# STLABTW/ST-DADK

Hardware: NVIDIA B200
Metric: train_samples_per_s (higher is better)
Workload: dtype tf32

## Files before the change

st_dadk_b200/csrc/api.cu:

```cuda
#include <cstdarg>
#include <cstdio>
#include <cstring>

#include "layer.cuh"
#include "misc.cuh"
#include "sparse.cuh"
#include "predict.cuh"
#include "field.cuh"

using namespace stdadk;

static thread_local char g_err[512] = "";

static int fail(int code, const char* fmt, ...) {
    va_list ap;
    va_start(ap, fmt);
    vsnprintf(g_err, sizeof(g_err), fmt, ap);
    va_end(ap);
    return code;
}
static int check_launch(const char* what) {
    cudaError_t e = cudaGetLastError();
    if (e != cudaSuccess) return fail((int)e, "%s: %s", what, cudaGetErrorString(e));
    return 0;
// ... 715 lines not shown
    K->p_cov = a->p_cov;
    K->fn = a->basis_fn;
    return 0;
}

static int make_groups(int n_groups, const int64_t* group_end, int64_t n, GroupsP* G) {
    REQUIRE(n_groups >= 1 && n_groups <= 8 && group_end, "optimizer: 1..8 parameter groups supported, got %d", n_groups);
    int64_t prev = 0;
    for (int i = 0; i < n_groups; ++i) {
        REQUIRE(group_end[i] >= prev, "optimizer: group_end must be non-decreasing");
        G->end[i] = prev = group_end[i];
    }
    REQUIRE(prev == n, "optimizer: last group_end (%lld) != n (%lld)", (long long)prev, (long long)n);
    G->n = n_groups;
    return 0;
}

size_t stdadk_celllist_ws_bytes(int32_t k_s, int32_t n_levels) {
    if (k_s < 0 || n_levels < 1 || n_levels > SP_MAX_LEVELS) return 0;
    return celllist_bytes(k_s, n_levels);
}

int stdadk_celllist_build(const float* knots4, int32_t k_s, const int32_t* level_begin, int32_t n_levels, void* ws,
                          size_t ws_bytes, void* stream) {
    if (int r = check_device()) return r;
    REQUIRE(knots4 && level_begin && ws && k_s >= 1, "celllist_build: NULL argument / no knots");
    REQUIRE(n_levels >= 1 && n_levels <= SP_MAX_LEVELS, "celllist_build: 1..%d levels, got %d", SP_MAX_LEVELS, n_levels);
    REQUIRE(((reinterpret_cast<uintptr_t>(ws) | reinterpret_cast<uintptr_t>(knots4)) & 15) == 0,
            "celllist_build: knots4 / workspace must be 16-byte aligned");
    REQUIRE(ws_bytes >= celllist_bytes(k_s, n_levels), "celllist_build: workspace of %zu B, need %zu B", ws_bytes,
            celllist_bytes(k_s, n_levels));
    CellBuildK K{};
    K.knots = reinterpret_cast<const float4*>(knots4);
    K.k_s = k_s;
    K.n_levels = n_levels;
    for (int l = 0; l <= n_levels; ++l) {
        REQUIRE(level_begin[l] >= (l ? level_begin[l - 1] : 0) && level_begin[l] <= k_s, "celllist_build: level_begin not monotone");
        K.level_begin[l] = level_begin[l];
    }
    REQUIRE(level_begin[0] == 0 && level_begin[n_levels] == k_s, "celllist_build: levels must cover [0, k_s)");
    K.ws = static_cast<int*>(ws);
    size_t ib = (celllist_ints(k_s, n_levels) * 4 + 15) & ~(size_t)15;
    K.sorted = reinterpret_cast<float4*>(static_cast<uint8_t*>(ws) + ib);
    celllist_build_kernel<<<1, CL_THREADS, 0, (cudaStream_t)stream>>>(K);
    return check_launch("celllist_build");
}

size_t stdadk_sqnorm_ws_floats(void) { return (size_t)SQNORM_BLOCKS * 8 + 8; }

int stdadk_grad_sqnorm(const float* g, int64_t n, int n_groups, const int64_t* group_end, float* sqnorms,
                       float* workspace, void* stream) {
    if (int r = check_device()) return r;
    REQUIRE(g && sqnorms && workspace && n > 0, "grad_sqnorm: bad arguments (workspace of stdadk_sqnorm_ws_floats() "
            "zero-initialised floats is required)");
    REQUIRE((reinterpret_cast<uintptr_t>(g) & 15) == 0, "grad_sqnorm: g must be 16-byte aligned");
    GroupsP G{};
    if (int r = make_groups(n_groups, group_end, n, &G)) return r;
    long long blocks = ((n >> 2) + SQNORM_THREADS * 4 - 1) / (SQNORM_THREADS * 4);
    if (blocks < 1) blocks = 1;
    if (blocks > SQNORM_BLOCKS) blocks = SQNORM_BLOCKS;
    sqnorm_kernel<<<(int)blocks, SQNORM_THREADS, 0, (cudaStream_t)stream>>>(g, n, G, sqnorms, workspace);
    return check_launch("grad_sqnorm");
}

int stdadk_sparse_l1_fwd(const stdadk_sparse_args* a, void* stream) {
    if (int r = check_device()) return r;
    SparseK K{};
    if (int r = sparse_fill(a, &K, false)) return r;
    if (a->pts.n_rows <= 0) return 0;
    int blocks = grid_for(a->pts.n_rows, SP_WARPS, 8);
    sparse_spatial_fwd_kernel<<<blocks, SP_WARPS * 32, 0, (cudaStream_t)stream>>>(K);
    return check_launch("sparse_l1_fwd");
}

int stdadk_sparse_l1_wgrad(const stdadk_sparse_args* a, void* stream) {
    if (int r = check_device()) return r;
    SparseK K{};
    if (int r = sparse_fill(a, &K, true)) return r;
    if (a->pts.n_rows <= 0) return 0;
    int blocks = grid_for(a->pts.n_rows, SP_WARPS, 8);
    sparse_spatial_wgrad_kernel<<<blocks, SP_WARPS * 32, 0, (cudaStream_t)stream>>>(K);
    return check_launch("sparse_l1_wgrad");
}

__global__ void step_inc_kernel(int* c) { *c += 1; }

int stdadk_peer_allreduce(const stdadk_peer_allreduce_args* a, void* stream) {
    if (int r = check_device()) return r;
    REQUIRE(a && a->g && a->step_count, "peer_allreduce: NULL argument");
    REQUIRE(a->world >= 2 && a->world <= PEER_MAX && a->rank >= 0 && a->rank < a->world,
            "peer_allreduce: world=%d rank=%d outside [2,%d]", a->world, a->rank, PEER_MAX);
    REQUIRE(a->n > 0 && a->n % 4 == 0, "peer_allreduce: n=%lld must be a positive multiple of 4", (long long)a->n);
    static_assert(PEER_MAX == STDADK_MAX_PEERS, "peer limits differ");
    REQUIRE((reinterpret_cast<uintptr_t>(a->g) & 15) == 0, "peer_allreduce: g must be 16-byte aligned");
    PeerK K{};
    for (int r = 0; r < a->world; ++r) {
        REQUIRE(a->recv[r] && (reinterpret_cast<uintptr_t>(a->recv[r]) & 15) == 0,
                "peer_allreduce: rank %d receive area not mapped / not 16-byte aligned", r);
        K.recv[r] = static_cast<uint4*>(a->recv[r]);
    }
    K.g = a->g;
    K.n2 = a->n / 2;
    K.step_count = a->step_count;
    K.rank = a->rank;
    K.world = a->world;
    REQUIRE(a->mode >= 0 && a->mode <= 2, "peer_allreduce: mode=%d (0 automatic, 1 one-shot, 2 two-phase)", a->mode);
    K.two_phase = a->mode == 2 || (a->mode == 0 && a->world >= 4);
    if (a->n_groups > 0) {
        REQUIRE(a->group_end && a->sqnorms && a->workspace, "peer_allreduce: fused norm needs group_end / sqnorms / workspace");
        K.n_norm = a->group_end[a->n_groups - 1];
        REQUIRE(K.n_norm <= a->n, "peer_allreduce: norm range exceeds n");
        if (int r = make_groups(a->n_groups, a->group_end, K.n_norm, &K.G)) return r;
        K.sq_out = a->sqnorms;
        K.ws = a->workspace;
    }
    long long blocks = (K.n2 + PEER_THREADS * 2 - 1) / (PEER_THREADS * 2);
    if (blocks > 148) blocks = 148;
    if (blocks < 1) blocks = 1;
    peer_allreduce_kernel<<<(int)blocks, PEER_THREADS, 0, (cudaStream_t)stream>>>(K);
    return check_launch("peer_allreduce");
}

int stdadk_adamw_ema_step(const stdadk_adamw_args* a, void* stream) {
    if (int r = check_device()) return r;
    REQUIRE(a && a->p && a->g && a->m && a->v && a->hyper && a->step_count && a->n > 0, "adamw: bad arguments");
    AdamK K{};
    if (int r = make_groups(a->n_groups, a->group_end, a->n, &K.G)) return r;
    K.p = a->p;
    K.g = a->g;
    K.m = a->m;
    K.v = a->v;
    K.shadow = a->shadow;
    K.n = a->n;
    K.hyper = a->hyper;
    K.sqnorms = a->sqnorms;
    K.step_count = a->step_count;
    K.beta1 = a->beta1;
    K.beta2 = a->beta2;
    K.eps = a->eps;
    K.ema_decay = a->ema_decay;
    K.g_zero = a->zero_grad ? const_cast<float*>(a->g) : nullptr;
    K.loss_acc = a->loss_acc;
    K.loss_sum = a->loss_sum;
    K.loss_last = a->loss_last;
    REQUIRE(((reinterpret_cast<uintptr_t>(a->p) | reinterpret_cast<uintptr_t>(a->g) | reinterpret_cast<uintptr_t>(a->m) |
              reinterpret_cast<uintptr_t>(a->v) | reinterpret_cast<uintptr_t>(a->shadow)) & 15) == 0,
            "adamw: buffers must be 16-byte aligned");
    if (a->fuse_norm) {
        REQUIRE(a->norm_ws, "adamw: fuse_norm needs norm_ws");
        K.sq_out = const_cast<float*>(a->sqnorms);
        K.norm_ws = a->norm_ws;
        K.step_rw = a->step_count;
        long long blocks = ((a->n + 3) / 4 + 255) / 256;
        if (blocks > 148) blocks = 148;
        const int sms = g_sm_count > 0 ? g_sm_count : 148;
        if (blocks > sms) blocks = sms;
        if (blocks < 1) blocks = 1;
        adamw_ema_kernel<true><<<(int)blocks, 256, 0, (cudaStream_t)stream>>>(K);
        return check_launch("adamw_ema_step (fused tail)");
    }
    step_inc_kernel<<<1, 1, 0, (cudaStream_t)stream>>>(a->step_count);
    adamw_ema_kernel<false><<<grid_for((a->n + 3) / 4, 256, 8), 256, 0, (cudaStream_t)stream>>>(K);
    return check_launch("adamw_ema_step");
}

}
```

st_dadk_b200/csrc/misc.cuh:

```cuda
#pragma once
#include "common.cuh"

namespace stdadk {

__global__ void pack_image_kernel(const float* __restrict__ src, long long row_stride, long long col_stride,
                                  long long rows, long long cols, float* __restrict__ img, long long n_chunks,
                                  int slabs) {
    for (long long idx = blockIdx.x * (long long)blockDim.x + threadIdx.x; idx < n_chunks;
         idx += (long long)gridDim.x * blockDim.x) {
        int chunk = (int)(idx & 7);
        int row = (int)((idx >> 3) & 127);
        long long ts = idx >> 10;
        int slab = (int)(ts % slabs);
        long long tile = ts / slabs;
        long long r = tile * TILE_M + row;
        float v[4];
#pragma unroll
        for (int e = 0; e < 4; ++e) {
            long long c = (long long)slab * SLAB_K + chunk * 4 + e;
            v[e] = (r < rows && c < cols) ? to_tf32(src[r * row_stride + c * col_stride]) : 0.0f;
        }
        float* dst = img + ts * SLAB_FLOATS;
        *reinterpret_cast<float4*>(reinterpret_cast<uint8_t*>(dst) + swz_off((uint32_t)row, (uint32_t)chunk)) =
            make_float4(v[0], v[1], v[2], v[3]);
// ... 197 lines not shown
}
constexpr int PEER_THREADS = 256;
__device__ __forceinline__ void peer_two_phase(const PeerK& P, unsigned int epoch, long long par_off, long long i0,
                                               long long stride) {
    float2* g2 = reinterpret_cast<float2*>(P.g);
    const long long m = (P.n2 + P.world - 1) / P.world;
    const long long own_lo = (long long)P.rank * m, own_hi = min(P.n2, own_lo + m);
    const uint4* mine = P.recv[P.rank];
    for (long long i = i0; i < P.n2; i += stride) {
        if (i >= own_lo && i < own_hi) continue;
        const int owner = (int)(i / m);
        const float2 v = g2[i];
        uint4* dst = nullptr;
#pragma unroll
        for (int p = 0; p < PEER_MAX; ++p)
            if (p == owner) dst = P.recv[p];
        st_sys_v4(dst + (par_off + P.rank) * P.n2 + i, make_uint4(__float_as_uint(v.x), epoch, __float_as_uint(v.y), epoch));
    }
    for (long long i = i0; i < P.n2; i += stride) {
        if (i < own_lo || i >= own_hi) continue;
        const float2 own = g2[i];
        float2 sum = make_float2(0.0f, 0.0f);
#pragma unroll
        for (int s = 0; s < PEER_MAX; ++s)
            if (s < P.world) {
                const float2 v = s == P.rank ? own : peer_wait_packet(mine + (par_off + s) * P.n2 + i, epoch);
                sum.x += v.x;
                sum.y += v.y;
            }
        g2[i] = sum;
        const uint4 pkt = make_uint4(__float_as_uint(sum.x), epoch, __float_as_uint(sum.y), epoch);
#pragma unroll
        for (int p = 0; p < PEER_MAX; ++p)
            if (p < P.world && p != P.rank) st_sys_v4(P.recv[p] + (par_off + P.rank) * P.n2 + i, pkt);
    }
    for (long long i = i0; i < P.n2; i += stride) {
        if (i >= own_lo && i < own_hi) continue;
        const int owner = (int)(i / m);
        g2[i] = peer_wait_packet(mine + (par_off + owner) * P.n2 + i, epoch);
    }
}
__global__ void __launch_bounds__(PEER_THREADS) peer_allreduce_kernel(const __grid_constant__ PeerK P) {
    const unsigned int epoch = (unsigned int)(*P.step_count) + 1u;
    const long long par_off = (long long)(epoch & 1u) * P.world;
    const long long stride = (long long)gridDim.x * blockDim.x;
    const long long i0 = blockIdx.x * (long long)blockDim.x + threadIdx.x;
    float2* g2 = reinterpret_cast<float2*>(P.g);
    float acc[8];
#pragma unroll
    for (int k = 0; k < 8; ++k) acc[k] = 0.0f;
    if (P.two_phase) {
        peer_two_phase(P, epoch, par_off, i0, stride);
        if (P.G.n == 0) return;
        for (long long i = i0; i < P.n2; i += stride) {
            const float2 sum = g2[i];
            const long long e = i << 1;
            const float vv[2] = {sum.x, sum.y};
#pragma unroll
            for (int j = 0; j < 2; ++j)
                if (e + j < P.n_norm) {
                    const int gi = group_of(P.G, e + j);
#pragma unroll
                    for (int k = 0; k < 8; ++k)
                        if (k == gi) acc[k] = fmaf(vv[j], vv[j], acc[k]);
                }
        }
    } else {
    for (long long i = i0; i < P.n2; i += stride) {
        const float2 v = g2[i];
        const uint4 pkt = make_uint4(__float_as_uint(v.x), epoch, __float_as_uint(v.y), epoch);
#pragma unroll
        for (int p = 0; p < PEER_MAX; ++p)
            if (p < P.world && p != P.rank) st_sys_v4(P.recv[p] + (par_off + P.rank) * P.n2 + i, pkt);
    }
    const uint4* mine = P.recv[P.rank];
    for (long long i = i0; i < P.n2; i += stride) {
        const float2 own = g2[i];
        float2 sum = make_float2(0.0f, 0.0f);
#pragma unroll
        for (int s = 0; s < PEER_MAX; ++s)
            if (s < P.world) {
                float2 v = own;
                if (s != P.rank) v = peer_wait_packet(mine + (par_off + s) * P.n2 + i, epoch);
                sum.x += v.x;
                sum.y += v.y;
            }
        g2[i] = sum;
        if (P.G.n > 0) {
            const long long e = i << 1;
            const float vv[2] = {sum.x, sum.y};
#pragma unroll
            for (int j = 0; j < 2; ++j)
                if (e + j < P.n_norm) {
                    const int gi = group_of(P.G, e + j);
#pragma unroll
                    for (int k = 0; k < 8; ++k)
                        if (k == gi) acc[k] = fmaf(vv[j], vv[j], acc[k]);
                }
        }
    }
    }
    if (P.G.n == 0) return;
    __shared__ float wsum[PEER_THREADS / 32][8];
    __shared__ bool last;
    const int warp = threadIdx.x >> 5, lane = threadIdx.x & 31;
#pragma unroll
    for (int k = 0; k < 8; ++k) {
        float s = warp_sum(acc[k]);
        if (lane == 0) wsum[warp][k] = s;
    }
    __syncthreads();
    if (threadIdx.x < 8) {
        float s = 0.0f;
        for (int w = 0; w < PEER_THREADS / 32; ++w) s += wsum[w][threadIdx.x];
        P.ws[blockIdx.x * 8 + threadIdx.x] = s;
    }
    __threadfence();
    __syncthreads();
    if (threadIdx.x == 0) {
        unsigned int* ticket = reinterpret_cast<unsigned int*>(P.ws + gridDim.x * 8);
        unsigned int t = atomicAdd(ticket, 1u);
        last = (t == gridDim.x - 1);
        if (last) *ticket = 0u;
    }
    __syncthreads();
    if (last && threadIdx.x < P.G.n) {
        __threadfence();
        float s = 0.0f;
        for (unsigned int b = 0; b < gridDim.x; ++b) s += P.ws[b * 8 + threadIdx.x];
        P.sq_out[threadIdx.x] = s;
    }
}

struct AdamK {
    float* p;
    const float* g;
    float* m;
    float* v;
    float* shadow;
    long long n;
    GroupsP G;
    const float* hyper;
    const float* sqnorms;
    const int* step_count;
    float beta1, beta2, eps, ema_decay;
    float* g_zero;
    float* loss_acc;
    float* loss_sum;
    float* loss_last;
    float* sq_out;
    float* norm_ws;
    int* step_rw;
};
template <bool FUSED>
__global__ void __launch_bounds__(256) adamw_ema_kernel(AdamK A) {
    __shared__ float s_sq[8];
    int step;
    if (FUSED) {
        step = *A.step_count + 1;
        float acc[8];
#pragma unroll
        for (int k = 0; k < 8; ++k) acc[k] = 0.0f;
        if (A.sqnorms) {
            const long long n4q = A.n >> 2;
            const float4* gq = reinterpret_cast<const float4*>(A.g);
            for (long long i = blockIdx.x * (long long)blockDim.x + threadIdx.x; i < n4q; i += (long long)gridDim.x * blockDim.x) {
                const float4 v = __ldg(gq + i);
                const long long e = i << 2;
                const float vv[4] = {v.x, v.y, v.z, v.w};
#pragma unroll
                for (int j = 0; j < 4; ++j) {
                    const int gi = group_of(A.G, e + j);
#pragma unroll
                    for (int k = 0; k < 8; ++k)
                        if (k == gi) acc[k] = fmaf(vv[j], vv[j], acc[k]);
                }
            }
            if (blockIdx.x == 0 && threadIdx.x < (A.n & 3)) {
                const long long i = (n4q << 2) + threadIdx.x;
                const float v = A.g[i];
                const int gi = group_of(A.G, i);
#pragma unroll
                for (int k = 0; k < 8; ++k)
                    if (k == gi) acc[k] = fmaf(v, v, acc[k]);
            }
        }
        __shared__ float wsum[8][8];
        const int warp = threadIdx.x >> 5, lane = threadIdx.x & 31;
#pragma unroll
        for (int k = 0; k < 8; ++k) {
            const float sk = warp_sum(acc[k]);
            if (lane == 0) wsum[warp][k] = sk;
        }
        __syncthreads();
        if (threadIdx.x < 8) {
            float sk = 0.0f;
            for (int w = 0; w < 8; ++w) sk += wsum[w][threadIdx.x];
            A.norm_ws[blockIdx.x * 8 + threadIdx.x] = sk;
        }
        __threadfence();
        __syncthreads();
        if (threadIdx.x == 0) {
            unsigned int* cnt = reinterpret_cast<unsigned int*>(A.norm_ws + gridDim.x * 8);
            volatile unsigned int* gen = cnt + 1;
            const unsigned int my_gen = *gen;
            if (atomicAdd(cnt, 1u) == gridDim.x - 1) {
                *cnt = 0u;
                __threadfence();
                atomicAdd(const_cast<unsigned int*>(gen), 1u);
            } else {
                long long t0 = clock64();
                while (*gen == my_gen) {
                    if (clock64() - t0 > 4000000000LL) __trap();
                }
            }
            __threadfence();
        }
        __syncthreads();
        if (threadIdx.x < 8) {
            float sk = 0.0f;
            for (unsigned int b = 0; b < gridDim.x; ++b) sk += __ldcg(&A.norm_ws[b * 8 + threadIdx.x]);
            s_sq[threadIdx.x] = sk;
            if (blockIdx.x == 0 && A.sq_out && threadIdx.x < A.G.n) A.sq_out[threadIdx.x] = sk;
        }
        if (blockIdx.x == 0 && threadIdx.x == 0) *A.step_rw = step;
        __syncthreads();
    } else {
        step = *A.step_count;
    }
    const float bc1 = 1.0f - powf(A.beta1, (float)step);
    const float bc2 = 1.0f - powf(A.beta2, (float)step);
    const float inv_sqrt_bc2 = 1.0f / sqrtf(bc2);
    float lr[8], wd[8], clip[8];
#pragma unroll
    for (int k = 0; k < 8; ++k) {
        lr[k] = wd[k] = 0.0f;
        clip[k] = 1.0f;
        if (k < A.G.n) {
            lr[k] = A.hyper[4 * k];
            wd[k] = A.hyper[4 * k + 1];
            float mx = A.hyper[4 * k + 2];
            if (A.sqnorms && mx > 0.0f) clip[k] = fminf(1.0f, mx / (sqrtf(FUSED ? s_sq[k] : A.sqnorms[k]) + 1e-6f));
        }
    }
    auto update = [&](long long i, float g, float& p, float& m, float& v, float& sh) {
        int gi = group_of(A.G, i);
        float l = lr[0], w = wd[0], c = clip[0];
#pragma unroll
        for (int k = 1; k < 8; ++k)
            if (k == gi) { l = lr[k]; w = wd[k]; c = clip[k]; }
        g *= c;
        p *= (1.0f - l * w);
        m = A.beta1 * m + (1.0f - A.beta1) * g;
        v = A.beta2 * v + (1.0f - A.beta2) * g * g;
        float denom = sqrtf(v) * inv_sqrt_bc2 + A.eps;
        p -= (l / bc1) * (m / denom);
        sh = A.ema_decay * sh + (1.0f - A.ema_decay) * p;
    };
    const long long n4 = A.n >> 2;
    const float4* g4 = reinterpret_cast<const float4*>(A.g);
    float4* p4 = reinterpret_cast<float4*>(A.p);
    float4* m4 = reinterpret_cast<float4*>(A.m);
    float4* v4 = reinterpret_cast<float4*>(A.v);
    float4* s4 = reinterpret_cast<float4*>(A.shadow);
    for (long long i = blockIdx.x * (long long)blockDim.x + threadIdx.x; i < n4;
         i += (long long)gridDim.x * blockDim.x) {
        float4 g = __ldg(g4 + i), p = p4[i], m = m4[i], v = v4[i];
        float4 sh = s4 ? s4[i] : make_float4(0.f, 0.f, 0.f, 0.f);
        const long long e = i << 2;
        update(e, g.x, p.x, m.x, v.x, sh.x);
        update(e + 1, g.y, p.y, m.y, v.y, sh.y);
        update(e + 2, g.z, p.z, m.z, v.z, sh.z);
        update(e + 3, g.w, p.w, m.w, v.w, sh.w);
        p4[i] = p;
        m4[i] = m;
        v4[i] = v;
        if (s4) s4[i] = sh;
        if (A.g_zero) reinterpret_cast<float4*>(A.g_zero)[i] = make_float4(0.f, 0.f, 0.f, 0.f);
    }
    if (blockIdx.x == 0 && threadIdx.x == 0 && A.loss_acc && A.loss_sum) {
        const float step_loss = *A.loss_acc;
        *A.loss_sum += step_loss;
        if (A.loss_last) *A.loss_last = step_loss;
        *A.loss_acc = 0.0f;
    }
    if (blockIdx.x == 0 && threadIdx.x < (A.n & 3)) {
        long long i = (n4 << 2) + threadIdx.x;
        float p = A.p[i], m = A.m[i], v = A.v[i], sh = A.shadow ? A.shadow[i] : 0.0f;
        update(i, A.g[i], p, m, v, sh);
        A.p[i] = p;
        A.m[i] = m;
        A.v[i] = v;
        if (A.shadow) A.shadow[i] = sh;
        if (A.g_zero) A.g_zero[i] = 0.0f;
    }
}

}
```

st_dadk_b200/trainer.py:

```python
from __future__ import annotations

import math
import os
import warnings
from dataclasses import dataclass
from typing import Dict, List, Optional

import numpy as np
import torch
import torch.distributed as dist

import threading

from . import _lib as L
from . import ops
from .executor import Executor, LossSpec, NetSpec


def _dist_on() -> bool:
    return dist.is_available() and dist.is_initialized() and dist.get_world_size() > 1


_CAPTURE_LOCK = threading.Lock()


class FlatState:

    def __init__(self, model, device):
        self.model = model
        blocks = model.hidden_blocks()
        entries = []
        for lin, ln in blocks:
            entries.append((lin.weight, (lin.in_features, lin.out_features), True))
            entries.append((lin.bias, tuple(lin.bias.shape), False))
            if ln is not None:
                entries.append((ln.weight, tuple(ln.weight.shape), False))
                entries.append((ln.bias, tuple(ln.bias.shape), False))
        if model.delta_params is not None:
            for d in model.delta_params:
                entries.append((d, tuple(d.shape), False))
        else:
            head = model.mlp[-1]
            entries.append((head.weight, tuple(head.weight.shape), False))
            entries.append((head.bias, tuple(head.bias.shape), False))
        n_mlp = sum(int(np.prod(s)) for _, s, _ in entries)
        sb = model.spatial_basis
        if sb.learnable:
            entries.append((sb.centers, tuple(sb.centers.shape), False))
            entries.append((sb.log_bandwidths, tuple(sb.log_bandwidths.shape), False))
        n = sum(int(np.prod(s)) for _, s, _ in entries)
        self.n = n
        self.group_end = [n_mlp, n] if sb.learnable else [n]
        q, d = model.output_dim, model.last_hidden_dim
        self.n_scratch = q * d + q if model.delta_params is not None else 0
        mk = lambda extra=0: torch.zeros(n + extra, dtype=torch.float32, device=device)
        self.p, self.m, self.v, self.shadow = mk(), mk(), mk(), mk()
        self.n_exchange = n + self.n_scratch + 1
        self.g = mk(self.n_scratch + 1 + (-self.n_exchange) % 4)
        self.loss_slot = self.g[n + self.n_scratch:n + self.n_scratch + 1]
        self.views: Dict[int, torch.Tensor] = {}
        self.gviews: Dict[int, torch.Tensor] = {}
        o = 0
        with torch.no_grad():
            for prm, shape, tr in entries:
                k = int(np.prod(shape))
                pv, gv = self.p[o:o + k].view(*shape), self.g[o:o + k].view(*shape)
                if tr:
                    pv, gv = pv.t(), gv.t()
                pv.copy_(prm.detach().to(device))
                prm.data = pv
                prm.grad = None
                self.views[id(prm)] = pv
                self.gviews[id(prm)] = gv
                o += k
        self.shadow.copy_(self.p)
        self._backup = None
        if self.n_scratch:
            self.g_head_w = self.g[n:n + q * d].view(q, d)
            self.g_head_b = self.g[n + q * d:n + q * d + q]

    def grad_views_for(self, model) -> dict:
        blocks = model.hidden_blocks()
        gv = self.gviews
        out = {"weights": [gv[id(l.weight)] for l, _ in blocks], "biases": [gv[id(l.bias)] for l, _ in blocks],
               "gammas": [gv[id(n.weight)] if n is not None else None for _, n in blocks],
               "betas": [gv[id(n.bias)] if n is not None else None for _, n in blocks]}
        if model.delta_params is not None:
            out["head_w"], out["head_b"] = self.g_head_w, self.g_head_b
        else:
            out["head_w"], out["head_b"] = gv[id(model.mlp[-1].weight)], gv[id(model.mlp[-1].bias)]
        sb = model.spatial_basis
        if sb.learnable:
            out["centers"], out["log_bandwidths"] = gv[id(sb.centers)], gv[id(sb.log_bandwidths)]
        else:
            out["centers"] = out["log_bandwidths"] = None
        return out

    def apply_shadow(self):
        self._backup = self.p.clone()
        self.p.copy_(self.shadow)

    def restore(self):
        self.p.copy_(self._backup)
        self._backup = None


@dataclass
class StepStats:
    loss: float
    n_rows: int


class Trainer:

    def __init__(self, model, config: dict, device, batches_per_epoch: int = 1, use_cuda_graph: bool = False):
        self.model = model.to(device)
        self.cfg = config
        if config.get("precision") is not None:
            self.model.precision = config["precision"]
        self.device = torch.device(device)
        if self.device.type != "cuda":
            raise RuntimeError("st_dadk_b200.Trainer runs on CUDA (sm_100) only; there is no CPU training path")
        self.flat = FlatState(self.model, self.device)
        self._peer = None
        if _dist_on() and dist.get_backend() == "nccl" and os.environ.get("STDADK_PEER_ALLREDUCE", "1") != "0":
            ok = torch.ones(1, device=self.device)
            try:
                from .peer import PeerExchange
                self._peer = PeerExchange(self.device, self.flat.n_exchange)
            except Exception as e:
                if "exceeds the peer-exchange limit" not in str(e):
                    warnings.warn(f"peer-memory gradient exchange unavailable ({e!r}); using the NCCL all-reduce")
                ok.zero_()
            dist.all_reduce(ok, op=dist.ReduceOp.MIN)
            if float(ok.item()) == 0.0:
                self._peer = None
        m = self.model
        self.learnable = bool(m.spatial_basis.learnable)
        self.q = m.output_dim
        self.head_w = torch.empty(self.q, m.last_hidden_dim, device=self.device)
        self.head_b = torch.empty(self.q, device=self.device)
        self.ex = Executor(self._spec())
        self.ex.loss_acc = self.flat.loss_slot
        self.ex.on_evict = lambda: self._graphs.clear()
        self.ex.alloc_grads(self.flat.g, self.flat.grad_views_for(m))
        self._init_loss()
        self._init_optimizer(batches_per_epoch)
        self.step_count = torch.zeros(1, dtype=torch.int32, device=self.device)
        self.sqnorms = torch.zeros(len(self.flat.group_end), device=self.device)
        self._sqnorm_ws = torch.zeros(L.lib().stdadk_sqnorm_ws_floats(), device=self.device)
        self._tail_ws = torch.zeros(148 * 8 + 8, device=self.device)
        self.seed = int(torch.initial_seed() & (2 ** 63 - 1))
        self.loss_sum = torch.zeros(1, device=self.device)
        self.loss_last = torch.zeros(1, device=self.device)
        self._g_clean = False
        self.use_cuda_graph = use_cuda_graph
        self._graphs: Dict[tuple, torch.cuda.CUDAGraph] = {}
        self._stage_idx = None
        self._host_stage = None
        self._host_perm = None
        self.world = dist.get_world_size() if _dist_on() else 1
        self.rank = dist.get_rank() if _dist_on() else 0
        c = self.cfg
        self._param_terms_possible = bool(
            self.learnable
            or (c.get("sparsity_penalty_type", "none") != "none"
                and (float(c.get("sparsity_lambda_l1", 0.001)) != 0.0 or float(c.get("sparsity_lambda_group", 0.01)) != 0.0))
            or (c.get("use_delta_reparameterization", False) and float(c.get("non_crossing_lambda", 0.0)) > 0))
        self.kernel_launches = 0

    def _spec(self) -> NetSpec:
        m = self.model
        self._refresh_head()
        return m.net_spec(self.head_w, self.head_b)

    def _refresh_head(self):
        m = self.model
        with torch.no_grad():
            if m.delta_params is not None:
                beta = torch.cumsum(torch.stack([d.detach() for d in m.delta_params]), dim=0)
                self.head_w.copy_(beta[:, 1:])
                self.head_b.copy_(beta[:, 0])
            else:
                self.head_w.copy_(m.mlp[-1].weight.detach())
                self.head_b.copy_(m.mlp[-1].bias.detach())

    def _init_loss(self):
        c = self.cfg
        rt = c.get("regression_type", "mean")
        if rt == "mean":
            self.loss = LossSpec("mse")
        elif rt == "quantile":
            if c.get("current_quantile") is None:
                raise ValueError("current_quantile must be specified for quantile regression")
            self.loss = LossSpec("pinball", [float(c["current_quantile"])])
        elif rt == "multi-quantile":
            taus = [float(x) for x in c.get("quantile_levels", [0.1, 0.5, 0.9])]
            ncw = 0.0 if c.get("use_delta_reparameterization", False) else float(c.get("non_crossing_weight", 0.0))
            self.loss = LossSpec("pinball", taus, ncw, int(c.get("non_crossing_power", 1)))
        else:
            raise ValueError(f"Unknown regression_type: {rt}")

    def _init_optimizer(self, batches_per_epoch: int):
        c = self.cfg
        self.lr = float(c.get("lr", 1e-3))
        self.wd = float(c.get("weight_decay", 1e-5))
        self.clip = float(c.get("grad_clip", 0) or 0)
        self.unfreeze_epoch = int(c.get("basis_unfreeze_epoch", 0))
        self.rampup_epochs = int(c.get("basis_lr_rampup_epochs", 0))
        dummy = lambda: [torch.nn.Parameter(torch.zeros(1))]
        if self.learnable:
            ratio = c.get("basis_lr_ratio", 0.05)
            init_basis = 0.0 if self.unfreeze_epoch > 0 else self.lr * ratio
            self.opt = torch.optim.AdamW([{"params": dummy(), "lr": self.lr, "name": "mlp"},
                                          {"params": dummy(), "lr": init_basis, "name": "basis"}], weight_decay=self.wd)
            for gq in self.opt.param_groups:
                gq["initial_lr"] = gq["lr"]
                if gq.get("name") == "basis":
                    gq["target_lr"] = self.lr * ratio
        else:
            self.opt = torch.optim.AdamW(dummy(), lr=self.lr, weight_decay=self.wd)
            for gq in self.opt.param_groups:
                gq["initial_lr"] = gq["lr"]
        self.batches_per_epoch = max(1, batches_per_epoch)
        self.warmup_epochs = int(c.get("warmup_epochs", 0))
        self.warmup_steps = self.warmup_epochs * self.batches_per_epoch if self.warmup_epochs > 0 else 0
        self.scheduler = None
        if c.get("scheduler") == "cosine":
            self.scheduler = torch.optim.lr_scheduler.CosineAnnealingLR(self.opt, T_max=c.get("epochs", 100),
                                                                        eta_min=self.lr * 0.5)
        self.ema_decay = 1.0 - 1.0 / (10.0 * self.batches_per_epoch)
        self.global_step = 0
        ng = len(self.opt.param_groups)
        self._hyper_ring = [torch.zeros(ng, 4, dtype=torch.float32).pin_memory() for _ in range(self.HYPER_SLOTS)]
        self._hyper_ev = [None] * self.HYPER_SLOTS
        self._hyper_k = 0
        self._hyper_last = None
        self.hyper = torch.zeros(ng, 4, dtype=torch.float32, device=self.device)

    HYPER_SLOTS = 16

    def _hyper_values(self):
        rows = []
        for gq in self.opt.param_groups:
            clip = self.clip * (0.1 if (self.learnable and gq.get("name") == "basis") else 1.0)
            rows.append((float(gq["lr"]), float(self.wd), float(clip)))
        return tuple(rows)

    def _push_hyper(self):
        vals = self._hyper_values()
        if vals == self._hyper_last:
            return
        k = self._hyper_k
        self._hyper_k = (k + 1) % self.HYPER_SLOTS
        if self._hyper_ev[k] is not None:
            self._hyper_ev[k].synchronize()
        slot = self._hyper_ring[k]
        for i, (lr, wd, clip) in enumerate(vals):
            slot[i, 0], slot[i, 1], slot[i, 2] = lr, wd, clip
        self.hyper.copy_(slot, non_blocking=True)
        ev = torch.cuda.Event()
        ev.record(torch.cuda.current_stream())
        self._hyper_ev[k] = ev
        self._hyper_last = vals

    def begin_epoch(self, epoch: int):
        if not (self.learnable and self.unfreeze_epoch > 0):
            return
        for gq in self.opt.param_groups:
            if gq.get("name") != "basis":
                continue
            if epoch == self.unfreeze_epoch:
                gq["lr"] = gq["target_lr"] * (0.1 if self.rampup_epochs > 0 else 1.0)
            elif self.unfreeze_epoch < epoch < self.unfreeze_epoch + self.rampup_epochs:
                gq["lr"] = gq["target_lr"] * (0.1 + 0.9 * (epoch - self.unfreeze_epoch) / self.rampup_epochs)

    def end_epoch(self, epoch: int):
        if self.scheduler is not None and epoch >= self.warmup_epochs:
            with warnings.catch_warnings():
                warnings.simplefilter("ignore")
                self.scheduler.step()

    def _penalty_terms(self):
        c, m = self.cfg, self.model
        terms = []
        if self.learnable:
            w = float(c.get("domain_penalty_weight", 0.0))
            if w > 0:
                terms.append(w * m.compute_domain_penalty())
            w = float(c.get("movement_penalty_weight", 0.0))
            if w > 0:
                terms.append(w * m.compute_movement_penalty())
        stype = c.get("sparsity_penalty_type", "none")
        l1, lg = float(c.get("sparsity_lambda_l1", 0.001)), float(c.get("sparsity_lambda_group", 0.01))
        if stype != "none" and (l1 != 0.0 or lg != 0.0):
            pen = m.compute_sparsity_penalty(penalty_type=stype, lambda_l1=l1, lambda_group=lg)
            if c.get("sparsity_apply_to_spatial", True):
                terms.append(pen["spatial_penalty"])
            if c.get("sparsity_apply_to_temporal", True):
                terms.append(pen["temporal_penalty"])
        if c.get("regression_type") == "multi-quantile" and c.get("use_delta_reparameterization", False):
            lam = float(c.get("non_crossing_lambda", 0.0))
            if lam > 0 and m.delta_params is not None and len(m.delta_params) > 1:
                pnc = 0.0
                for d in list(m.delta_params)[1:]:
                    pnc = pnc + d[0] - torch.max(d[0], torch.clamp(-d[1:], min=0.0).sum())
                terms.append(lam * pnc)
        return terms

    def _add_penalty_grads(self):
        terms = self._penalty_terms()
        if not terms:
            return None
        total = sum(terms)
        params = [p for p in self.model.parameters() if p.requires_grad]
        sb = self.model.spatial_basis
        sb._hook_enabled = False
        try:
            grads = torch.autograd.grad(total, params, allow_unused=True)
        finally:
            sb._hook_enabled = True
        for p, gr in zip(params, grads):
            if gr is not None:
                self.flat.gviews[id(p)].add_(gr)
        return total.detach()

    def _finish_special_grads(self):
        m = self.model
        if m.delta_params is not None:
            dbeta = torch.cat([self.flat.g_head_b[:, None], self.flat.g_head_w], dim=1)
            ddelta = torch.flip(torch.cumsum(torch.flip(dbeta, [0]), dim=0), [0])
            for k, d in enumerate(m.delta_params):
                self.flat.gviews[id(d)].copy_(ddelta[k])

    def _damp_center_grads(self):
        sb = self.model.spatial_basis
        if self.learnable and sb.gradient_damping:
            gv = self.flat.gviews[id(sb.centers)]
            gv.copy_(sb._damping_factor() * gv)

    def _step_compute(self, table, perm, row_begin: int, n_rows: int, global_rows: int, key_offset: int = 0):
        ex, fl = self.ex, self.flat
        if not self._g_clean:
            fl.g.zero_()
            ex.loss_acc.zero_()
        self._g_clean = False
        self._refresh_head()
        ex.prepare(force=True, for_backward=True)
        pts = ops.make_points(table.coords, table.t, table.X, index=perm, row_begin=row_begin, n_rows=n_rows)
        ex.forward(pts, train=True, seed=self.seed, y=table.y, loss=self.loss, inv_count=1.0 / (global_rows * self.q),
                   save=True, prepared=True, step_ptr=self.step_count, key_offset=key_offset)
        ex.backward(zero=False)
        self._finish_special_grads()

    def _step_exchange(self):
        if self.world > 1:
            if self._peer is not None:
                fuse = self._norm_fused()
                self._peer.allreduce(self.flat.g, self.step_count, self.flat.group_end if fuse else None, self.sqnorms)
            else:
                dist.all_reduce(self.flat.g[:self.flat.n_exchange])

    def _norm_fused(self) -> bool:
        return self._peer is not None and self.world > 1 and self.clip > 0 and not self._param_terms_possible

    def _step_update(self):
        ex, fl = self.ex, self.flat
        pen = self._add_penalty_grads()
        self._damp_center_grads()
        fused_tail = not self._norm_fused()
        scratch_tail = fl.n_scratch > 0
        ops.adamw_ema_step(fl.p, fl.g[:fl.n], fl.m, fl.v, fl.shadow, fl.group_end, self.hyper,
                           self.sqnorms if self.clip > 0 else None, self.step_count, ema_decay=self.ema_decay,
                           zero_grad=True, loss_acc=ex.loss_acc, loss_sum=self.loss_sum, loss_last=self.loss_last,
                           norm_ws=self._tail_ws if fused_tail else None)
        if scratch_tail:
            fl.g[fl.n:fl.n + fl.n_scratch].zero_()
        self._g_clean = True
        if pen is not None:
            self.loss_sum += pen

    def _step_body(self, table, perm, row_begin: int, n_rows: int, global_rows: int, key_offset: int = 0):
        self._step_compute(table, perm, row_begin, n_rows, global_rows, key_offset)
        self._step_exchange()
        self._step_update()

    def train_step(self, table, perm: torch.Tensor, row_begin: int, n_rows: int, global_rows: Optional[int] = None,
                   key_offset: Optional[int] = None):
        if global_rows is None:
            global_rows = n_rows
        if key_offset is None:
            key_offset = shard_rows(global_rows, self.rank, self.world)[0] if self.world > 1 else 0
        self._push_hyper()
        if self.use_cuda_graph:
            if self._stage_idx is None or self._stage_idx.shape[0] < n_rows:
                self._stage_idx = torch.zeros(max(n_rows, 1), dtype=torch.int64, device=self.device)
                self._graphs.clear()
            self._stage_idx[:n_rows].copy_(perm[row_begin:row_begin + n_rows])
            gkey = (n_rows, global_rows, table.coords.data_ptr(), table.t.data_ptr(), table.y.data_ptr(),
                    table.X.data_ptr() if table.X is not None else 0, key_offset)
            g = self._graphs.get(gkey)
            if g is None:
                with _CAPTURE_LOCK:
                    self._step_body(table, self._stage_idx, 0, n_rows, global_rows, key_offset)
                    torch.cuda.current_stream().synchronize()
                    mode = dict(capture_error_mode="thread_local")
                    one_graph = self.world == 1 or self._peer is not None
                    if one_graph:
                        g1 = torch.cuda.CUDAGraph()
                        with torch.cuda.graph(g1, **mode):
                            self._step_body(table, self._stage_idx, 0, n_rows, global_rows, key_offset)
                        g = (g1, None)
                    else:
                        g1, g2 = torch.cuda.CUDAGraph(), torch.cuda.CUDAGraph()
                        with torch.cuda.graph(g1, **mode):
                            self._step_compute(table, self._stage_idx, 0, n_rows, global_rows, key_offset)
                        with torch.cuda.graph(g2, **mode):
                            self._step_update()
                        g = (g1, g2)
                self._graphs[gkey] = g
            else:
                g[0].replay()
                if g[1] is not None:
                    self._step_exchange()
                    g[1].replay()
        else:
            self._step_body(table, perm, row_begin, n_rows, global_rows, key_offset)
        if self.global_step < self.warmup_steps:
            f = (self.global_step + 1) / self.warmup_steps
            for gq in self.opt.param_groups:
                gq["lr"] = gq["initial_lr"] * f
        self.global_step += 1

    def train_step_host(self, host_table, row_begin: int, n_rows: int, global_rows: Optional[int] = None,
                        lagged: bool = False) -> float:
        if self._host_stage is None or len(self._host_stage[0]) < n_rows:
            from stnf.dataio import ObservationTable
            z = lambda *sh: torch.zeros(*sh, dtype=torch.float32, device=self.device)
            mk = lambda: ObservationTable(z(n_rows, 2), z(n_rows), z(n_rows),
                                          z(n_rows, self.model.p) if self.model.p > 0 else None)
            self._host_stage = [mk(), mk()]
            self._graphs.clear()
            self._host_perm = torch.arange(n_rows, dtype=torch.int64, device=self.device)
            self._host_copy_stream = torch.cuda.Stream(device=self.device)
            self._host_ready = [torch.cuda.Event(), torch.cuda.Event()]
            self._host_done = [torch.cuda.Event(), torch.cuda.Event()]
            self._host_loss = [torch.full((1,), float("nan")).pin_memory(), torch.full((1,), float("nan")).pin_memory()]
            self._host_k = 0
            self._host_pending = None
            main = torch.cuda.current_stream()
            for e in self._host_done:
                e.record(main)
        k = self._host_k
        self._host_k ^= 1
        st = self._host_stage[k]
        sl = slice(row_begin, row_begin + n_rows)
        main = torch.cuda.current_stream()

        def copy_batch():
            st.coords[:n_rows].copy_(host_table.coords[sl], non_blocking=True)
            st.t[:n_rows].copy_(host_table.t[sl], non_blocking=True)
            st.y[:n_rows].copy_(host_table.y[sl], non_blocking=True)
            if st.X is not None:
                st.X[:n_rows].copy_(host_table.X[sl], non_blocking=True)

        if lagged or self._host_pending is not None:
            with torch.cuda.stream(self._host_copy_stream):
                self._host_copy_stream.wait_event(self._host_done[k])
                copy_batch()
                self._host_ready[k].record(self._host_copy_stream)
            main.wait_event(self._host_ready[k])
        else:
            copy_batch()
        self.train_step(st, self._host_perm, 0, n_rows, global_rows)
        self._host_loss[k].copy_(self.loss_last, non_blocking=True)
        self._host_done[k].record(main)
        prev, self._host_pending = self._host_pending, k
        if not lagged:
            self._host_done[k].synchronize()
            self._host_pending = None
            return float(self._host_loss[k].item())
        if prev is None:
            return float("nan")
        self._host_done[prev].synchronize()
        return float(self._host_loss[prev].item())

    def flush_host_loss(self) -> float:
        if self._host_pending is None:
            return float("nan")
        k, self._host_pending = self._host_pending, None
        self._host_done[k].synchronize()
        return float(self._host_loss[k].item())

    @property
    def launches_per_step(self) -> int:
        nh = self.ex.spec.n_hidden
        n = 1
        n += nh + nh + nh
        if self.learnable:
            n += 3
        n += 1 if not self._norm_fused() else 2
        if self._peer is not None and self.world > 1:
            n += 1
        return n

    def profile_step(self, table, perm, n_rows: int, global_rows: int, repeats: int = 10) -> dict:
        rec: List[tuple] = []
        saved = {}

        def wrap(name, fn, flops_of):
            def inner(*a, **k):
                e0, e1 = torch.cuda.Event(enable_timing=True), torch.cuda.Event(enable_timing=True)
                e0.record()
                r = fn(*a, **k)
                e1.record()
                rec.append((name(*a, **k) if callable(name) else name, e0, e1, flops_of(*a, **k)))
                return r
            return inner

        rows = float(n_rows)
        f_fwd = lambda a: 2.0 * rows * a.layer.n_in * a.layer.n_out
        f_bwd = lambda a: 2.0 * rows * a.layer.n_out * (a.layer.n_in + (a.n_next if not a.head else 0))
        f_wg = lambda a: 2.0 * rows * a.n_in * a.n_out
        patches = {
            "layer_fwd": (lambda a: f"layer_fwd[{a.layer.layer_id}]", f_fwd),
            "layer_bwd": (lambda a: f"layer_bwd[{a.layer.layer_id}]", f_bwd),
            "wgrad": (lambda a: f"wgrad[{a.n_in}x{a.n_out}]", f_wg),
            "knot_grad": ("knot_grad", lambda a: 2.0 * rows * a.n_out * self.model.k_spatial),
            "pack_image": ("pack_image", lambda *a, **k: 0.0),
            "pack_images": ("pack_images", lambda *a, **k: 0.0),
            "knots_prepare": ("knots_prepare", lambda *a, **k: 0.0),
            "tknots_prepare": ("knots_prepare", lambda *a, **k: 0.0),
            "grad_sqnorm": ("grad_sqnorm", lambda *a, **k: 0.0),
            "adamw_ema_step": ("adamw_ema_step", lambda *a, **k: 0.0),
        }
        use_graph, self.use_cuda_graph = self.use_cuda_graph, False
        try:
            for fname, (nm, fl) in patches.items():
                saved[fname] = getattr(ops, fname)
                setattr(ops, fname, wrap(nm, saved[fname], fl))
            self.train_step(table, perm, 0, n_rows, global_rows)
            rec.clear()
            s0, s1 = torch.cuda.Event(enable_timing=True), torch.cuda.Event(enable_timing=True)
            s0.record()
            for i in range(repeats):
                self.train_step(table, perm, (i + 1) * n_rows, n_rows, global_rows)
            s1.record()
            torch.cuda.synchronize()
        finally:
            for fname, fn in saved.items():
                setattr(ops, fname, fn)
            self.use_cuda_graph = use_graph
        agg: Dict[str, dict] = {}
        for name, e0, e1, fl in rec:
            d = agg.setdefault(name, {"ms": 0.0, "count": 0, "flops": fl})
            d["ms"] += e0.elapsed_time(e1)
            d["count"] += 1
        for d in agg.values():
            d["count"] = d["count"] / repeats
            d["ms"] = d["ms"] / (d["count"] * repeats)
        return {"kernels": agg, "step_ms": sum(d["ms"] * d["count"] for d in agg.values()),
                "eager_step_ms_wall": s0.elapsed_time(s1) / repeats}

    def pop_loss_sum(self) -> float:
        v = float(self.loss_sum.item())
        self.loss_sum.zero_()
        return v

    @torch.no_grad()
    def evaluate(self, table, batch_rows: int = 65536, with_loss: bool = True):
        ex = self.ex
        n = len(table)
        out = torch.empty(n, self.q, device=self.device)
        self._refresh_head()
        ex.prepare(force=True, for_backward=False)
        losses = []
        for b in range(0, n, batch_rows):
            r = min(batch_rows, n - b)
# ... 122 lines not shown
```

Measured before the change: 24.43 million.

## Cache optimizer tail operands in registers and double-buffer index staging on side stream

In the fused AdamW+EMA tail, each thread now loads its g/p/m/v/shadow vectors into registers once when the grid covers the parameters, and reuses them for both the grad-norm pass and the update instead of reading from global memory twice. Per-block partial norms are staged through shared memory, and the hyperparameter loads are hoisted above the grid barrier. On the Python side, the perm-index copy goes into one of two staging buffers on a separate stream with events, so it can overlap the previous graph replay. The head weights alias the model parameters when no delta params exist, which removes a per-step copy. In exchange, the change doubles the number of captured graphs and adds register pressure and stream-synchronization complexity.

```diff
diff --git a/st_dadk_b200/csrc/api.cu b/st_dadk_b200/csrc/api.cu
--- a/st_dadk_b200/csrc/api.cu
+++ b/st_dadk_b200/csrc/api.cu
@@ -891,7 +891,7 @@
         K.norm_ws = a->norm_ws;
         K.step_rw = a->step_count;
         long long blocks = ((a->n + 3) / 4 + 255) / 256;
-        if (blocks > 148) blocks = 148;
+        if (blocks > TAIL_MAX_BLOCKS) blocks = TAIL_MAX_BLOCKS;
         const int sms = g_sm_count > 0 ? g_sm_count : 148;
         if (blocks > sms) blocks = sms;
         if (blocks < 1) blocks = 1;
diff --git a/st_dadk_b200/csrc/misc.cuh b/st_dadk_b200/csrc/misc.cuh
--- a/st_dadk_b200/csrc/misc.cuh
+++ b/st_dadk_b200/csrc/misc.cuh
@@ -373,32 +373,71 @@
     float* norm_ws;
     int* step_rw;
 };
+constexpr int TAIL_MAX_BLOCKS = 148;
+constexpr int TAIL_REG_VECS = 2;
 template <bool FUSED>
 __global__ void __launch_bounds__(256) adamw_ema_kernel(AdamK A) {
     __shared__ float s_sq[8];
     int step;
+    const long long n4 = A.n >> 2;
+    const long long stride = (long long)gridDim.x * blockDim.x;
+    const long long i0 = blockIdx.x * (long long)blockDim.x + threadIdx.x;
+    const float4* g4 = reinterpret_cast<const float4*>(A.g);
+    float4* p4 = reinterpret_cast<float4*>(A.p);
+    float4* m4 = reinterpret_cast<float4*>(A.m);
+    float4* v4 = reinterpret_cast<float4*>(A.v);
+    float4* s4 = reinterpret_cast<float4*>(A.shadow);
+    const bool in_regs = FUSED && n4 <= TAIL_REG_VECS * stride;
+    float4 rg[TAIL_REG_VECS], rp[TAIL_REG_VECS], rm[TAIL_REG_VECS], rv[TAIL_REG_VECS], rs[TAIL_REG_VECS];
+    if (in_regs) {
+#pragma unroll
+        for (int r = 0; r < TAIL_REG_VECS; ++r) {
+            const long long i = i0 + r * stride;
+            if (i < n4) {
+                rg[r] = __ldg(g4 + i);
+                rp[r] = p4[i];
+                rm[r] = m4[i];
+                rv[r] = v4[i];
+                rs[r] = s4 ? s4[i] : make_float4(0.f, 0.f, 0.f, 0.f);
+            }
+        }
+    }
+    float lr[8], wd[8], mx[8];
+#pragma unroll
+    for (int k = 0; k < 8; ++k) {
+        lr[k] = wd[k] = mx[k] = 0.0f;
+        if (k < A.G.n) {
+            lr[k] = A.hyper[4 * k];
+            wd[k] = A.hyper[4 * k + 1];
+            mx[k] = A.hyper[4 * k + 2];
+        }
+    }
     if (FUSED) {
         step = *A.step_count + 1;
         float acc[8];
 #pragma unroll
         for (int k = 0; k < 8; ++k) acc[k] = 0.0f;
+        auto add_sq = [&](long long i, const float4 v) {
+            const long long e = i << 2;
+            const float vv[4] = {v.x, v.y, v.z, v.w};
+#pragma unroll
+            for (int j = 0; j < 4; ++j) {
+                const int gi = group_of(A.G, e + j);
+#pragma unroll
+                for (int k = 0; k < 8; ++k)
+                    if (k == gi) acc[k] = fmaf(vv[j], vv[j], acc[k]);
+            }
+        };
         if (A.sqnorms) {
-            const long long n4q = A.n >> 2;
-            const float4* gq = reinterpret_cast<const float4*>(A.g);
-            for (long long i = blockIdx.x * (long long)blockDim.x + threadIdx.x; i < n4q; i += (long long)gridDim.x * blockDim.x) {
-                const float4 v = __ldg(gq + i);
-                const long long e = i << 2;
-                const float vv[4] = {v.x, v.y, v.z, v.w};
-#pragma unroll
-                for (int j = 0; j < 4; ++j) {
-                    const int gi = group_of(A.G, e + j);
-#pragma unroll
-                    for (int k = 0; k < 8; ++k)
-                        if (k == gi) acc[k] = fmaf(vv[j], vv[j], acc[k]);
-                }
+            if (in_regs) {
+#pragma unroll
+                for (int r = 0; r < TAIL_REG_VECS; ++r)
+                    if (i0 + r * stride < n4) add_sq(i0 + r * stride, rg[r]);
+            } else {
+                for (long long i = i0; i < n4; i += stride) add_sq(i, __ldg(g4 + i));
             }
             if (blockIdx.x == 0 && threadIdx.x < (A.n & 3)) {
-                const long long i = (n4q << 2) + threadIdx.x;
+                const long long i = (n4 << 2) + threadIdx.x;
                 const float v = A.g[i];
                 const int gi = group_of(A.G, i);
 #pragma unroll
@@ -438,9 +477,12 @@
             __threadfence();
         }
         __syncthreads();
+        __shared__ float s_part[TAIL_MAX_BLOCKS * 8];
+        for (unsigned int q = threadIdx.x; q < gridDim.x * 8; q += blockDim.x) s_part[q] = __ldcg(&A.norm_ws[q]);
+        __syncthreads();
         if (threadIdx.x < 8) {
             float sk = 0.0f;
-            for (unsigned int b = 0; b < gridDim.x; ++b) sk += __ldcg(&A.norm_ws[b * 8 + threadIdx.x]);
+            for (unsigned int b = 0; b < gridDim.x; ++b) sk += s_part[b * 8 + threadIdx.x];
             s_sq[threadIdx.x] = sk;
             if (blockIdx.x == 0 && A.sq_out && threadIdx.x < A.G.n) A.sq_out[threadIdx.x] = sk;
         }
@@ -452,17 +494,12 @@
     const float bc1 = 1.0f - powf(A.beta1, (float)step);
     const float bc2 = 1.0f - powf(A.beta2, (float)step);
     const float inv_sqrt_bc2 = 1.0f / sqrtf(bc2);
-    float lr[8], wd[8], clip[8];
+    float clip[8];
 #pragma unroll
     for (int k = 0; k < 8; ++k) {
-        lr[k] = wd[k] = 0.0f;
         clip[k] = 1.0f;
-        if (k < A.G.n) {
-            lr[k] = A.hyper[4 * k];
-            wd[k] = A.hyper[4 * k + 1];
-            float mx = A.hyper[4 * k + 2];
-            if (A.sqnorms && mx > 0.0f) clip[k] = fminf(1.0f, mx / (sqrtf(FUSED ? s_sq[k] : A.sqnorms[k]) + 1e-6f));
-        }
+        if (k < A.G.n && A.sqnorms && mx[k] > 0.0f)
+            clip[k] = fminf(1.0f, mx[k] / (sqrtf(FUSED ? s_sq[k] : A.sqnorms[k]) + 1e-6f));
     }
     auto update = [&](long long i, float g, float& p, float& m, float& v, float& sh) {
         int gi = group_of(A.G, i);
@@ -478,16 +515,7 @@
         p -= (l / bc1) * (m / denom);
         sh = A.ema_decay * sh + (1.0f - A.ema_decay) * p;
     };
-    const long long n4 = A.n >> 2;
-    const float4* g4 = reinterpret_cast<const float4*>(A.g);
-    float4* p4 = reinterpret_cast<float4*>(A.p);
-    float4* m4 = reinterpret_cast<float4*>(A.m);
-    float4* v4 = reinterpret_cast<float4*>(A.v);
-    float4* s4 = reinterpret_cast<float4*>(A.shadow);
-    for (long long i = blockIdx.x * (long long)blockDim.x + threadIdx.x; i < n4;
-         i += (long long)gridDim.x * blockDim.x) {
-        float4 g = __ldg(g4 + i), p = p4[i], m = m4[i], v = v4[i];
-        float4 sh = s4 ? s4[i] : make_float4(0.f, 0.f, 0.f, 0.f);
+    auto update4 = [&](long long i, float4 g, float4 p, float4 m, float4 v, float4 sh) {
         const long long e = i << 2;
         update(e, g.x, p.x, m.x, v.x, sh.x);
         update(e + 1, g.y, p.y, m.y, v.y, sh.y);
@@ -498,6 +526,14 @@
         v4[i] = v;
         if (s4) s4[i] = sh;
         if (A.g_zero) reinterpret_cast<float4*>(A.g_zero)[i] = make_float4(0.f, 0.f, 0.f, 0.f);
+    };
+    if (in_regs) {
+#pragma unroll
+        for (int r = 0; r < TAIL_REG_VECS; ++r)
+            if (i0 + r * stride < n4) update4(i0 + r * stride, rg[r], rp[r], rm[r], rv[r], rs[r]);
+    } else {
+        for (long long i = i0; i < n4; i += stride)
+            update4(i, __ldg(g4 + i), p4[i], m4[i], v4[i], s4 ? s4[i] : make_float4(0.f, 0.f, 0.f, 0.f));
     }
     if (blockIdx.x == 0 && threadIdx.x == 0 && A.loss_acc && A.loss_sum) {
         const float step_loss = *A.loss_acc;
diff --git a/st_dadk_b200/trainer.py b/st_dadk_b200/trainer.py
--- a/st_dadk_b200/trainer.py
+++ b/st_dadk_b200/trainer.py
@@ -138,8 +138,11 @@
         m = self.model
         self.learnable = bool(m.spatial_basis.learnable)
         self.q = m.output_dim
-        self.head_w = torch.empty(self.q, m.last_hidden_dim, device=self.device)
-        self.head_b = torch.empty(self.q, device=self.device)
+        if m.delta_params is None:
+            self.head_w, self.head_b = m.mlp[-1].weight.detach(), m.mlp[-1].bias.detach()
+        else:
+            self.head_w = torch.empty(self.q, m.last_hidden_dim, device=self.device)
+            self.head_b = torch.empty(self.q, device=self.device)
         self.ex = Executor(self._spec())
         self.ex.loss_acc = self.flat.loss_slot
         self.ex.on_evict = lambda: self._graphs.clear()
@@ -176,14 +179,11 @@
 
     def _refresh_head(self):
         m = self.model
-        with torch.no_grad():
-            if m.delta_params is not None:
+        if m.delta_params is not None:
+            with torch.no_grad():
                 beta = torch.cumsum(torch.stack([d.detach() for d in m.delta_params]), dim=0)
                 self.head_w.copy_(beta[:, 1:])
                 self.head_b.copy_(beta[:, 0])
-            else:
-                self.head_w.copy_(m.mlp[-1].weight.detach())
-                self.head_b.copy_(m.mlp[-1].bias.detach())
 
     def _init_loss(self):
         c = self.cfg
@@ -393,28 +393,46 @@
             key_offset = shard_rows(global_rows, self.rank, self.world)[0] if self.world > 1 else 0
         self._push_hyper()
         if self.use_cuda_graph:
-            if self._stage_idx is None or self._stage_idx.shape[0] < n_rows:
-                self._stage_idx = torch.zeros(max(n_rows, 1), dtype=torch.int64, device=self.device)
+            main = torch.cuda.current_stream()
+            if self._stage_idx is None or self._stage_idx[0].shape[0] < n_rows:
+                self._stage_idx = [torch.zeros(max(n_rows, 1), dtype=torch.int64, device=self.device) for _ in range(2)]
+                self._stage_stream = torch.cuda.Stream(device=self.device)
+                self._stage_read = [None, None]
+                self._stage_k = 0
+                self._stage_perm = None
                 self._graphs.clear()
-            self._stage_idx[:n_rows].copy_(perm[row_begin:row_begin + n_rows])
+            k = self._stage_k
+            self._stage_k ^= 1
+            side = self._stage_stream
+            perm_key = (perm.data_ptr(), perm._version, perm.shape[0])
+            if perm_key != self._stage_perm:
+                side.wait_stream(main)
+                self._stage_perm = perm_key
+            if self._stage_read[k] is not None:
+                side.wait_event(self._stage_read[k])
+            with torch.cuda.stream(side):
+                self._stage_idx[k][:n_rows].copy_(perm[row_begin:row_begin + n_rows])
+            perm.record_stream(side)
+            main.wait_stream(side)
+            stage = self._stage_idx[k]
             gkey = (n_rows, global_rows, table.coords.data_ptr(), table.t.data_ptr(), table.y.data_ptr(),
-                    table.X.data_ptr() if table.X is not None else 0, key_offset)
+                    table.X.data_ptr() if table.X is not None else 0, key_offset, k)
             g = self._graphs.get(gkey)
             if g is None:
                 with _CAPTURE_LOCK:
-                    self._step_body(table, self._stage_idx, 0, n_rows, global_rows, key_offset)
+                    self._step_body(table, stage, 0, n_rows, global_rows, key_offset)
                     torch.cuda.current_stream().synchronize()
                     mode = dict(capture_error_mode="thread_local")
                     one_graph = self.world == 1 or self._peer is not None
                     if one_graph:
                         g1 = torch.cuda.CUDAGraph()
                         with torch.cuda.graph(g1, **mode):
-                            self._step_body(table, self._stage_idx, 0, n_rows, global_rows, key_offset)
+                            self._step_body(table, stage, 0, n_rows, global_rows, key_offset)
                         g = (g1, None)
                     else:
                         g1, g2 = torch.cuda.CUDAGraph(), torch.cuda.CUDAGraph()
                         with torch.cuda.graph(g1, **mode):
-                            self._step_compute(table, self._stage_idx, 0, n_rows, global_rows, key_offset)
+                            self._step_compute(table, stage, 0, n_rows, global_rows, key_offset)
                         with torch.cuda.graph(g2, **mode):
                             self._step_update()
                         g = (g1, g2)
@@ -424,6 +442,9 @@
                 if g[1] is not None:
                     self._step_exchange()
                     g[1].replay()
+            ev = torch.cuda.Event()
+            ev.record(main)
+            self._stage_read[k] = ev
         else:
             self._step_body(table, perm, row_begin, n_rows, global_rows, key_offset)
         if self.global_step < self.warmup_steps:
```

New measurement: 24.71 million (median of 6 runs). 1.01x the previous value.
